# junhong-3dv/s2m2

Measured on AMD Instinct MI355X. Metric: stereo pairs/sec, S-model 1216x1024 fp16 refine_iter=3 (ms/pair = 1000*n_gpus/value), higher is better.
Workload: dtype f16; 1 GPU; S-model 1216x1024 refine_iter=3 use_positivity=True, 1 pair(s) per GPU per step, random-init weights (seeded LeCun normal); pairs_per_gpu=1, parallelism=dp1 (pairs sharded, RCCL gather of outputs to rank 0)

## Files before the change

### __graft_entry__.py

```python
import os
import sys

ROOT = os.path.dirname(os.path.abspath(__file__))
if ROOT not in sys.path:
    sys.path.insert(0, ROOT)


def build() -> None:
    from s2m2_amd.build import build as build_lib
    lib = build_lib(verbose=True)
    assert os.path.exists(lib)
    _check_isa()
    import s2m2_amd
    from s2m2_amd import hip
    hip.load()
    import oracle.s2m2_oracle
    _build_ref()
    print("[build] ok:", lib)


def _build_ref() -> None:
    from oracle import make_ref, ref_loader
    if os.path.isdir(make_ref.SRC):
        make_ref.build(verbose=True)
    print("[build] oracle/_ref:", "ok" if ref_loader.available() else f"absent ({ref_loader.why_not()})")


def _check_isa() -> None:
    from s2m2_amd import build as B
    csrc = os.path.join(ROOT, "s2m2_amd", "csrc")
    if "-DS2M2_UNTRACKED_LOADS=0" in B.effective_defines():
        print("[build] check_isa: skipped (tracked loads: nothing to guard)")
        return
    stamp = os.path.join(B.OBJ, f"check_isa.{B.config_key()}.ok")
    newest = max(os.path.getmtime(os.path.join(csrc, f)) for f in os.listdir(csrc) if f in ("conv.hip", "conv_narrow.hip", "fusion.hip", "ln_corr.hip", "convblock.hip", "convgru.hip") or f.endswith(".h"))
    newest = max(newest, os.path.getmtime(os.path.join(ROOT, "tools", "check_isa.py")))
    if os.path.exists(stamp) and os.path.getmtime(stamp) > newest:
        print("[build] check_isa: up to date")
        return
    import subprocess
    r = subprocess.run([sys.executable, os.path.join(ROOT, "tools", "check_isa.py")], capture_output=True, text=True)
    sys.stdout.write(r.stdout)
    if r.returncode != 0:
        if os.environ.get("S2M2_ISA_FALLBACK") == "1":
            print("[build] check_isa failed (assertions above): S2M2_ISA_FALLBACK=1 -> rebuilding with tracked loads (-DS2M2_UNTRACKED_LOADS=0)")
            B.build(force=True, verbose=True, extra_defines=("-DS2M2_UNTRACKED_LOADS=0",))
            return
        raise RuntimeError("tools/check_isa.py failed -- the violated assertions:\n" + r.stdout + r.stderr[-2000:] +
                           "\n(S2M2_ISA_FALLBACK=1 rebuilds the library with tracked loads instead of failing)")
    open(stamp, "w").write("ok\n")


def smoke() -> None:
    import torch
    from oracle import s2m2_oracle as O
    from s2m2_amd.model import S2M2
    from s2m2_amd.weights import seeded_state_dict, synthetic_pair
    assert torch.cuda.is_available(), "smoke() needs cuda:0"
    torch.cuda.set_device(0)
    sd = seeded_state_dict(128, 1, 1, 0)
    m = S2M2(128, 1, 1, use_positivity=True, refine_iter=1)
    m.load_state_dict(sd, strict=True)
    m = m.cuda().eval()
    left, right = synthetic_pair(64, 96, 1, 8, 0)
    cap = {}
    d, o, c = m(left.cuda(), right.cuda(), capture=cap)
    torch.cuda.synchronize()
    ocap = {}
# ... 17 lines not shown
```

### include/s2m2_hip.h

```cpp
#ifndef S2M2_HIP_H
#define S2M2_HIP_H

#include <stddef.h>
#include <stdint.h>

#ifdef __cplusplus
extern "C" {
#endif

enum { S2M2_F32 = 0, S2M2_F16 = 1 };

#define S2M2_ABI_VERSION 800
int s2m2_version(void);
const char* s2m2_last_error(void);
int s2m2_debug_poison_lds(void* stream);
int s2m2_debug_clock_probe(void* out, void* stream);

const char* s2m2_ln_corr_kernel_name(int C, int feat_dtype, int cv_dtype);

typedef struct s2m2_corr_desc {
    const void* tokens;
    const float* ln_weight;
    const float* ln_bias;
    void* cv;
// ... 160 lines not shown
    long long out_stride;
    int N, H, W, C;
    const void* w_conv0;
    const void* w_conv2;
    const void* w_1x0;
    const void* w_1x2;
    const float* b_conv0;
    const float* b_conv2;
    const float* b_1x0;
    const float* b_1x2;
    int patch_rows;
    int dtype;
} s2m2_convblock_desc;
int s2m2_conv_block_supported(int C, int H, int W, int dtype);
int s2m2_conv_block(const s2m2_convblock_desc* desc, void* stream);

typedef struct s2m2_convgru_desc {
    const void* h;
    long long h_stride;
    const void* x;
    long long x_stride;
    void* out;
    long long out_stride;
    int N, H, W, C;
    int KH, KW;
    const void* w_zr;
    const void* w_q;
    const float* b_zr;
    const float* b_q;
    int dtype;
} s2m2_convgru_desc;
int s2m2_conv_gru_supported(int C, int H, int W, int dtype);
int s2m2_conv_gru(const s2m2_convgru_desc* desc, void* stream);

typedef struct s2m2_pw_desc {
    const void* src[4];
    int src_c[4];
    long long src_stride[4];
    int nsrc;
    long long rows;
    const void* weight_frag;
    const float* bias;
    void* out;
    long long out_stride;
    int Cout;
    int act;
    int shuffle2, Ho, Wo;
    int dtype;
} s2m2_pw_desc;
int s2m2_pw_direct_supported(int K, int Cout, int dtype);
int s2m2_pw_direct(const s2m2_pw_desc* desc, void* stream);

typedef struct s2m2_narrow_desc {
    const void* x;
    long long x_stride;
    int N, H, W, Cin;
    const void* x1;
    long long x1_stride;
    int Cin1;
    const void* weight_frag;
    const float* bias;
    void* out;
    long long out_stride;
    int Cout, KH, KW, stride;
    int act;
    int dtype;
// ... 135 lines not shown
```

### s2m2_amd/csrc/plan.h

```cpp
#pragma once
#include <stddef.h>
#include <type_traits>
#include <vector>
#include "common.h"

namespace s2m2 {

bool plan_recording();
constexpr int kPlanMaskWords = 4;
struct PlanPtrMask {
    unsigned long long bits[kPlanMaskWords] = {0, 0, 0, 0};
    bool overflow = false;
    void set(size_t byte_off) {
        const size_t w = byte_off / 8;
        if (byte_off % 8 != 0 || w >= 64 * kPlanMaskWords) overflow = true;
        else bits[w / 64] |= 1ULL << (w % 64);
    }
    bool test(size_t w) const { return w < 64 * kPlanMaskWords && ((bits[w / 64] >> (w % 64)) & 1ULL) != 0; }
};
int plan_append(int (*tramp)(const void* blob, void* stream), const void* blob, size_t bytes, const char* name, const PlanPtrMask& mask);

struct PlanEntry {
    const char* name;
    int (*tramp)(const void* blob, void* stream);
// ... 60 lines not shown
}

template <typename D> struct PlanPtrFields;
#define S2M2_PLAN_PTRS(D, ...)                                                                                      \
    template <> struct PlanPtrFields<D> {                                                                           \
        static void mark(size_t base, PlanPtrMask& m) {                                                             \
            const size_t offs[] = {__VA_ARGS__};                                                                    \
            for (size_t o : offs) m.set(base + o);                                                                  \
        }                                                                                                           \
    };
#define S2M2_OFF(D, f) offsetof(D, f)
#define S2M2_OFF_I(D, f, i) (offsetof(D, f) + 8 * (i))
S2M2_PLAN_PTRS(s2m2_corr_desc, S2M2_OFF(s2m2_corr_desc, tokens), S2M2_OFF(s2m2_corr_desc, ln_weight), S2M2_OFF(s2m2_corr_desc, ln_bias),
               S2M2_OFF(s2m2_corr_desc, cv), S2M2_OFF(s2m2_corr_desc, start_event), S2M2_OFF(s2m2_corr_desc, stop_event))
S2M2_PLAN_PTRS(s2m2_conv_desc, S2M2_OFF_I(s2m2_conv_desc, src, 0), S2M2_OFF_I(s2m2_conv_desc, src, 1), S2M2_OFF_I(s2m2_conv_desc, src, 2),
               S2M2_OFF_I(s2m2_conv_desc, src, 3), S2M2_OFF(s2m2_conv_desc, weight), S2M2_OFF(s2m2_conv_desc, bias), S2M2_OFF(s2m2_conv_desc, out),
               S2M2_OFF(s2m2_conv_desc, aux0), S2M2_OFF(s2m2_conv_desc, aux1), S2M2_OFF(s2m2_conv_desc, ln_wsum), S2M2_OFF(s2m2_conv_desc, bias2))
S2M2_PLAN_PTRS(s2m2_chain_desc, S2M2_OFF(s2m2_chain_desc, x), S2M2_OFF(s2m2_chain_desc, res), S2M2_OFF(s2m2_chain_desc, out),
               S2M2_OFF_I(s2m2_chain_desc, weight, 0), S2M2_OFF_I(s2m2_chain_desc, weight, 1), S2M2_OFF_I(s2m2_chain_desc, weight, 2),
               S2M2_OFF_I(s2m2_chain_desc, bias, 0), S2M2_OFF_I(s2m2_chain_desc, bias, 1), S2M2_OFF_I(s2m2_chain_desc, bias, 2),
               S2M2_OFF_I(s2m2_chain_desc, ln_wsum, 0), S2M2_OFF_I(s2m2_chain_desc, ln_wsum, 1), S2M2_OFF_I(s2m2_chain_desc, ln_wsum, 2),
               S2M2_OFF(s2m2_chain_desc, ln_out), S2M2_OFF(s2m2_chain_desc, ln_gamma), S2M2_OFF(s2m2_chain_desc, ln_beta),
               S2M2_OFF(s2m2_chain_desc, fan_weight), S2M2_OFF(s2m2_chain_desc, fan_bias), S2M2_OFF(s2m2_chain_desc, fan_ln_wsum),
               S2M2_OFF(s2m2_chain_desc, fan_out))
S2M2_PLAN_PTRS(s2m2_rowattn_desc, S2M2_OFF(s2m2_rowattn_desc, x), S2M2_OFF(s2m2_rowattn_desc, out), S2M2_OFF(s2m2_rowattn_desc, weights),
               S2M2_OFF(s2m2_rowattn_desc, vectors), S2M2_OFF(s2m2_rowattn_desc, ln_out))
S2M2_PLAN_PTRS(s2m2_convblock_desc, S2M2_OFF(s2m2_convblock_desc, x), S2M2_OFF(s2m2_convblock_desc, out), S2M2_OFF(s2m2_convblock_desc, w_conv0),
               S2M2_OFF(s2m2_convblock_desc, w_conv2), S2M2_OFF(s2m2_convblock_desc, w_1x0), S2M2_OFF(s2m2_convblock_desc, w_1x2),
               S2M2_OFF(s2m2_convblock_desc, b_conv0), S2M2_OFF(s2m2_convblock_desc, b_conv2), S2M2_OFF(s2m2_convblock_desc, b_1x0),
               S2M2_OFF(s2m2_convblock_desc, b_1x2))
S2M2_PLAN_PTRS(s2m2_convgru_desc, S2M2_OFF(s2m2_convgru_desc, h), S2M2_OFF(s2m2_convgru_desc, x), S2M2_OFF(s2m2_convgru_desc, out),
               S2M2_OFF(s2m2_convgru_desc, w_zr), S2M2_OFF(s2m2_convgru_desc, w_q), S2M2_OFF(s2m2_convgru_desc, b_zr),
               S2M2_OFF(s2m2_convgru_desc, b_q))
S2M2_PLAN_PTRS(s2m2_pw_desc, S2M2_OFF_I(s2m2_pw_desc, src, 0), S2M2_OFF_I(s2m2_pw_desc, src, 1), S2M2_OFF_I(s2m2_pw_desc, src, 2),
               S2M2_OFF_I(s2m2_pw_desc, src, 3), S2M2_OFF(s2m2_pw_desc, weight_frag), S2M2_OFF(s2m2_pw_desc, bias), S2M2_OFF(s2m2_pw_desc, out))
S2M2_PLAN_PTRS(s2m2_narrow_desc, S2M2_OFF(s2m2_narrow_desc, x), S2M2_OFF(s2m2_narrow_desc, x1), S2M2_OFF(s2m2_narrow_desc, weight_frag),
               S2M2_OFF(s2m2_narrow_desc, bias), S2M2_OFF(s2m2_narrow_desc, out), S2M2_OFF(s2m2_narrow_desc, head_frag),
               S2M2_OFF(s2m2_narrow_desc, head_bias))

template <typename D> struct PlanDescBlob { int (*impl)(const D*, void*); D desc; };
template <typename D> int plan_desc_tramp(const void* blob, void* stream) {
    const auto* b = static_cast<const PlanDescBlob<D>*>(blob);
    return b->impl(&b->desc, stream);
}
template <typename D> int plan_dispatch_desc(const char* name, int (*impl)(const D*, void*), const D* d, void* stream) {
#if S2M2_RANGE_CHECK
    range_bind_tu();
    const int rc = impl(d, stream) || range_collect(name, stream);
#else
    const int rc = impl(d, stream);
#endif
    if (rc == 0 && d && plan_recording()) {
        PlanDescBlob<D> b;
        __builtin_memset(&b, 0, sizeof(b));
        b.impl = impl;
        b.desc = *d;
        PlanPtrMask m;
        PlanPtrFields<D>::mark(offsetof(PlanDescBlob<D>, desc), m);
        return plan_append(&plan_desc_tramp<D>, &b, sizeof(b), name, m);
    }
    return rc;
}

template <typename... T> struct TypeList {};
template <typename Done, typename... Rest> struct DropLast;
template <typename... D, typename L> struct DropLast<TypeList<D...>, L> { using type = TypeList<D...>; };
// ... 21 lines not shown
```

### s2m2_amd/engine.py

```python
from __future__ import annotations

import os
from dataclasses import dataclass
from functools import cached_property
from typing import Dict, Optional, Sequence, Tuple

import torch
import torch.nn.functional as F

from . import hip, pack

Tensor = torch.Tensor


@dataclass(eq=False)
class Layer:
    weight: Tensor
    bias: Optional[Tensor]
    kh: int
    kw: int
    cout: int
    korder: int = 0

    def __post_init__(self):
# ... 72 lines not shown
    return max(1, (MAX_PIXELS - 1) // (2 * H * W))


class Engine:
    def __init__(self, model, dtype: torch.dtype):
        hip.load()
        self.dtype = dtype
        self.C = model.feature_channels
        self.ntr = model.num_transformer
        self.use_positivity = model.use_positivity
        self.refine_iter = model.refine_iter
        self.output_upsample = model.output_upsample
        self.device = next(model.parameters()).device
        self.p: Dict[str, Tensor] = {n: q.detach().to(self.device, torch.float32) for n, q in model.named_parameters()}
        self._layers: Dict[object, Layer] = {}
        self._composites: Dict[object, object] = {}
        self._supported: Dict[tuple, object] = {}
        self._pe_cache: Dict[Tuple[int, int], Tuple[Tensor, Tensor]] = {}
        self._bufs: Dict[object, Tensor] = {}
        self._plans: Dict[object, object] = {}
        self._ns = None
        self.fuse_k1ln = os.environ.get("S2M2_FUSE_K1LN", "1") != "0"
        self.cv_band = 11 if (os.environ.get("S2M2_CV_BAND", "0") == "1" and self.use_positivity) else -1
        self.use_k12 = os.environ.get("S2M2_K12", "1") != "0"
        self.use_k12_head = self.use_k12 and os.environ.get("S2M2_K12_HEAD", "1") != "0"
        self.native_refine = os.environ.get("S2M2_REFINE_NATIVE", "1") != "0"
        self.use_rowfuse = os.environ.get("S2M2_ROWFUSE", "1") != "0"
        self.coarse_fuse = os.environ.get("S2M2_COARSE_FUSE", "1") != "0"
        self.use_convblock = os.environ.get("S2M2_CONVBLOCK", "1") != "0"
        self.convblock_maxpix = int(os.environ.get("S2M2_CONVBLOCK_MAXPIX", "40000"))
        self.convblock_c256 = os.environ.get("S2M2_CONVBLOCK_C256", "0") == "1"
        self.gru_frag = os.environ.get("S2M2_GRU_FRAG", "0") == "1"
        self.gru_fuse = os.environ.get("S2M2_GRU_FUSE", "1") != "0"
        self._tokens_normed: Optional[Tensor] = None
        self.ln_w = self.p["disp_init.layer_norm.weight"].contiguous()
        self.ln_b = self.p["disp_init.layer_norm.bias"].contiguous()
        self.k1_events = None

    def std(self, name: str, splits: Optional[Sequence[Tuple[int, int]]] = None, transposed: bool = False, frag: bool = True) -> Layer:
        key = (name, tuple(splits) if splits else None, transposed, bool(frag))
        s = self._layers.get(key)
        if s is None:
            w = self.p[name + ".weight"]
            if transposed:
                w = pack.convT_s1_as_conv(w)
            if w.dim() == 2:
                w = w[:, :, None, None]
            cin_p = sum(pd for _, pd in splits) if splits else pack.pad8(w.shape[1])
            frag = frag and pack.frag_eligible(pack.pad8(w.shape[0]), cin_p, w.shape[2], w.shape[3], self.dtype)
            wp = pack.pack_conv_frag(w, self.dtype, splits) if frag else pack.pack_conv(w, self.dtype, splits)
            s = self._layers[key] = Layer(wp, pack.pack_bias(self.p.get(name + ".bias"), w.shape[0]), w.shape[2], w.shape[3],
                                          pack.pad8(w.shape[0]), 2 if frag else 0)
        return s

    def merged(self, key: str, parts: Sequence[Tuple[str, int, float, bool]], cin_total: int) -> Layer:
        s = self._layers.get(key)
        if s is None:
            rows, biases = [], []
            kh = kw = 1
            for name, off, wscale, tr in parts:
                w = self.p[name + ".weight"]
                if tr:
                    w = pack.convT_s1_as_conv(w)
                if w.dim() == 2:
                    w = w[:, :, None, None]
                co, ci, kh, kw = w.shape
# ... 65 lines not shown
        b = self._bufs.get(k)
        if b is None:
            if self._ns is None and len(self._bufs) >= 64:
                self._bufs.pop(next(iter(self._bufs)))
            b = torch.zeros(shape, device=self.device, dtype=dtype or self.dtype)
            self._bufs[k] = b
        return b

    def down(self, p: str, x: Tensor) -> Tensor:
        spec = self.std(p + ".1")
        c = x.shape[-1]
        pooled = spec.is_1x1 and x.dim() == 4 and x.shape[1] >= 2 and x.shape[2] >= 2
        if pooled and (spec.plain_1x1(c, c) or spec.plain_1x1(c, 2 * c)) and self.chain_frag_ok(c):
            return hip.mlp_fan(x, *spec.fan(ln=False), pool2=True)
        if pooled:
            return self.cconv(spec, [x], pool2=True)
        return self.cconv(spec, [hip.resample2x(x, 0)])

    def up(self, p: str, x: Tensor) -> Tensor:
        spec = self.std(p + ".1")
        if spec.is_1x1:
            return hip.resample2x(self.cconv(spec, [x]), 1)
        return self.cconv(spec, [hip.resample2x(x, 1)])

    def conv_block(self, p: str, z: Tensor) -> Tensor:
        c0, c2 = self.std(p + ".convs_1x.0"), self.std(p + ".convs_1x.2")
        c = z.shape[-1]
        same = c0.cout == c and c2.cout == c
        if (self.use_convblock and same and z.dim() == 4 and z.shape[0] * z.shape[1] * z.shape[2] <= self.convblock_maxpix
                and (c == 128 or self.convblock_c256) and self.chain_frag_ok(c) and self.convblock_ok(c, z.shape[1], z.shape[2])):
            k0, k2 = self.std(p + ".convs.0"), self.std(p + ".convs.2")
            if k0.frag_3x3(c) and k2.frag_3x3(c) and c0.plain_1x1(c, c) and c2.plain_1x1(c, c):
                return hip.conv_block(z, k0.weight, k0.bias, k2.weight, k2.bias, c0.chain_frag, c0.bias, c2.chain_frag, c2.bias)
        if same and self.chain_frag_ok(c):
            b = hip.mlp_chain(z, [c0.stage(hip.ACT_RELU), c2.stage(hip.ACT_NONE)], frag=True)
        elif same and self.chain_ok(c):
            b = hip.mlp_chain(z, [c0.stage(hip.ACT_RELU, frag=False), c2.stage(hip.ACT_NONE, frag=False)])
        else:
            b = self.cconv(c2, [self.cconv(c0, [z], act=hip.ACT_RELU)])
        t = self.cconv(self.std(p + ".convs.0"), [z], act=hip.ACT_GELU)
        return self.cconv(self.std(p + ".convs.2"), [t], epi=hip.EPI_ADD, aux0=b)

    def gate_fusion(self, p: str, c: int) -> Layer:
        return self.merged(p + "|gate+fusion", [(p + ".feature_gate.0", 0, 1.0, False), (p + ".feature_fusion.0", 0, 1.0, False)], 2 * c)

    def dual_heads(self, p: str):
        def build():
            g2, f2 = self.std(p + ".feature_gate.2"), self.std(p + ".feature_fusion.2")
            return torch.cat([g2.weight, f2.weight], dim=1).contiguous(), g2.bias, f2.bias
        return self.composite(p + "|gate.2+fusion.2", build)

    def k10(self, p: str, z0: Tensor, z1: Tensor, first: Layer, z1_coarse: bool = False) -> Tensor:
        dual = self.dual_heads(p)
        if self.fusion_frag_ok(z0.shape[-1]):
            ws = self.composite(p + "|k10 fragment stream", lambda: pack.fusion_frag(first.weight, dual[0]))
            return hip.feature_fusion(z0, z1, ws, first.bias, None, dual[1], dual[2], z1_coarse=z1_coarse, frag=True)
        return hip.feature_fusion(z0, z1, first.weight, first.bias, dual[0], dual[1], dual[2], z1_coarse=z1_coarse)

    def fusion_up_ok(self, p: str, c: int, pu: str) -> bool:
        spec = self.std(pu + ".1")
        return (spec.is_1x1 and spec.cout == c and self.gate_fusion(p, c).is_1x1
                and self.p[p + ".feature_gate.0.weight"].shape[0] == c and self.fusion_ok(c))

    def up_tail(self, p: str, c_fine: int, pu: str, c_coarse: int) -> Optional[Layer]:
        spec = self.std(pu + ".1")
        if (self.coarse_fuse and self.fusion_up_ok(p, c_fine, pu) and spec.plain_1x1(c_coarse, c_coarse) and c_fine == c_coarse
# ... 12 lines not shown
        c = z0.shape[-1]
        cg = self.p[p + ".feature_gate.0.weight"].shape[0]
        spec = self.gate_fusion(p, c)
        if spec.is_1x1 and cg == c and self.fusion_ok(c):
            return self.k10(p, z0, z1, spec)
        gf = self.cconv(spec, [z0, z1], act=hip.ACT_GELU)
        if cg % 64 == 0:
            dual = self.dual_heads(p)
            return hip.conv2d([gf], dual[0], dual[1], 1, 1, dual[0].shape[0], act=hip.ACT_SIGMOID, epi=hip.EPI_DUALMIX, aux0=z0, aux1=z1,
                              ksplit=cg, bias2=dual[2])
        m = self.cconv(self.std(p + ".feature_gate.2"), [gf[..., :cg]], act=hip.ACT_SIGMOID, epi=hip.EPI_GATEMIX, aux0=z0, aux1=z1)
        return self.cconv(self.std(p + ".feature_fusion.2"), [gf[..., cg:]], epi=hip.EPI_ADD, aux0=m)

    def chain_ok(self, c: int) -> bool:
        return self.supported("mlp_chain", c)

    def chain_frag_ok(self, c: int) -> bool:
        return self.supported("mlp_chain_frag", c)

    def fusion_frag_ok(self, c: int) -> bool:
        return self.supported("feature_fusion_frag", c)

    def fusion_ok(self, c: int) -> bool:
        return self.supported("feature_fusion", c) or self.fusion_frag_ok(c)

    def pw_ok(self, k: int, cout: int) -> bool:
        return self.supported("pw_direct", k, cout)

    def narrow_ok(self, kh: int, kw: int, stride: int, cin: int, cout: int) -> bool:
        return self.use_k12 and self.supported("conv_narrow", kh, kw, stride, cin, cout)

    def gru_fuse_ok(self, c: int, h: int, w: int) -> bool:
        return getattr(hip, "conv_gru_supported", None) is not None and self.supported("conv_gru", c, h, w)

    def convblock_ok(self, c: int, h: int, w: int) -> bool:
        return self.supported("conv_block", c, h, w)

    def row_ok(self, z: Tensor, nh: int) -> bool:
        return self.use_rowfuse and z.dim() == 4 and self.supported("row_attn", z.shape[-1], nh, z.shape[2])

    def pe(self, h: int, w: int) -> Tuple[Tensor, Tensor]:
        key = (h, w)
        if key not in self._pe_cache:
            self._pe_cache[key] = pe_tables(h, w, self.device)
        return self._pe_cache[key]

    def qkv_spec(self, p: str) -> Layer:
        c = self.p[p + ".q.weight"].shape[1]
        return self.merged(p + "|qkv", [(p + ".q", 0, 1.0, False), (p + ".k", 0, 1.0, False), (p + ".v", 0, 1.0, False)], c)

    def qkv(self, p: str, x: Tensor) -> Tensor:
        spec = self.qkv_spec(p)
        c = x.shape[-1]
        if spec.is_1x1 and spec.cout == 3 * c and self.chain_frag_ok(c):
            return hip.mlp_fan(x, *spec.fan())
        return self.cconv(spec, [x], ln=True)

    def attn_core(self, p: str, z: Tensor, nh: int, two_d: bool, cross: bool, use_pe: bool, qkv: Optional[Tensor] = None) -> Tensor:
        n, h, w, c = z.shape
        if qkv is None:
            qkv = self.qkv(p + ".attn", z)
        v3 = qkv.reshape(n, h * w, 3 * c) if two_d else qkv.reshape(n * h, w, 3 * c)
        q, k, v = v3[..., :c], v3[..., c:2 * c], v3[..., 2 * c:]
        if use_pe:
            px, py = self.pe(h, w)
            o, pes = hip.attention(q, k, v, nh, pe=(px, py, w, h))
# ... 439 lines not shown
```

### s2m2_amd/hip.py

```python
from __future__ import annotations

import contextlib
import ctypes
import os
from typing import Optional, Tuple

import torch

_HERE = os.path.dirname(os.path.abspath(__file__))
LIB_PATH = os.path.join(_HERE, "lib", "libs2m2_hip%s.so" % os.environ.get("S2M2_LIB_SUFFIX", ""))

F32, F16 = 0, 1
_DT = {torch.float32: F32, torch.float16: F16}

_lib: Optional[ctypes.CDLL] = None

_vp, _i, _ll = ctypes.c_void_p, ctypes.c_int, ctypes.c_longlong

ACT_NONE, ACT_GELU, ACT_RELU, ACT_SIGMOID, ACT_TANH = 0, 1, 2, 3, 4
EPI_NONE, EPI_ADD, EPI_MUL, EPI_GRU, EPI_GATEMIX, EPI_DUALMIX = 0, 1, 2, 3, 4, 5


class ConvDesc(ctypes.Structure):
    _fields_ = [("src", _vp * 4), ("src_c", _i * 4), ("src_stride", _i * 4), ("nsrc", _i), ("weight", _vp), ("bias", _vp),
                ("out", _vp), ("out_stride", _i), ("N", _i), ("H", _i), ("W", _i), ("KH", _i), ("KW", _i), ("Cout", _i),
                ("act", _i), ("epi", _i), ("aux0", _vp), ("aux1", _vp), ("aux0_stride", _i), ("aux1_stride", _i),
                ("out_scale", ctypes.c_float), ("shuffle2", _i), ("tile", _i), ("dtype", _i), ("korder", _i), ("stride", _i),
                ("ln_wsum", _vp), ("ln_eps", ctypes.c_float), ("ksplit", _i), ("bias2", _vp), ("pool2", _i), ("epi_cout0", _i)]


class ChainDesc(ctypes.Structure):
    _fields_ = [("x", _vp), ("res", _vp), ("out", _vp), ("x_stride", _ll), ("res_stride", _ll), ("out_stride", _ll), ("rows", _ll),
                ("C", _i), ("nstage", _i), ("weight", _vp * 3), ("bias", _vp * 3), ("ln_wsum", _vp * 3), ("act", _i * 3),
                ("res_stage", _i), ("carry", _i), ("ln_eps", ctypes.c_float), ("dtype", _i),
                ("ln_out", _vp), ("ln_out_stride", _ll), ("ln_gamma", _vp), ("ln_beta", _vp), ("ln_out_eps", ctypes.c_float),
                ("fan_weight", _vp), ("fan_bias", _vp), ("fan_ln_wsum", _vp), ("fan_out", _vp), ("fan_out_stride", _ll),
                ("nfan", _i), ("xcd_group_rows", _ll), ("weight_frag", _i), ("pool_h", _i), ("pool_w", _i)]


class RowAttnDesc(ctypes.Structure):
    _fields_ = [("x", _vp), ("x_stride", _ll), ("out", _vp), ("out_stride", _ll), ("nimg", _i), ("h", _i), ("w", _i), ("C", _i), ("heads", _i),
                ("cross", _i), ("weights", _vp), ("vectors", _vp), ("ln_eps", ctypes.c_float),
                ("ln_out", _vp), ("ln_out_stride", _ll), ("ln_out_eps", ctypes.c_float), ("xcd_hint", _i), ("dtype", _i)]


class ConvBlockDesc(ctypes.Structure):
    _fields_ = [("x", _vp), ("x_stride", _ll), ("out", _vp), ("out_stride", _ll), ("N", _i), ("H", _i), ("W", _i), ("C", _i),
                ("w_conv0", _vp), ("w_conv2", _vp), ("w_1x0", _vp), ("w_1x2", _vp), ("b_conv0", _vp), ("b_conv2", _vp), ("b_1x0", _vp),
                ("b_1x2", _vp), ("patch_rows", _i), ("dtype", _i)]


class ConvGruDesc(ctypes.Structure):
    _fields_ = [("h", _vp), ("h_stride", _ll), ("x", _vp), ("x_stride", _ll), ("out", _vp), ("out_stride", _ll), ("N", _i), ("H", _i), ("W", _i),
                ("C", _i), ("KH", _i), ("KW", _i), ("w_zr", _vp), ("w_q", _vp), ("b_zr", _vp), ("b_q", _vp), ("dtype", _i)]


class PwDesc(ctypes.Structure):
    _fields_ = [("src", _vp * 4), ("src_c", _i * 4), ("src_stride", _ll * 4), ("nsrc", _i), ("rows", _ll), ("weight_frag", _vp), ("bias", _vp),
                ("out", _vp), ("out_stride", _ll), ("Cout", _i), ("act", _i), ("shuffle2", _i), ("Ho", _i), ("Wo", _i), ("dtype", _i)]


class NarrowDesc(ctypes.Structure):
    _fields_ = [("x", _vp), ("x_stride", _ll), ("N", _i), ("H", _i), ("W", _i), ("Cin", _i), ("x1", _vp), ("x1_stride", _ll), ("Cin1", _i),
                ("weight_frag", _vp), ("bias", _vp), ("out", _vp), ("out_stride", _ll), ("Cout", _i), ("KH", _i), ("KW", _i), ("stride", _i),
                ("act", _i), ("dtype", _i), ("head_frag", _vp), ("head_bias", _vp), ("head_cout", _i)]


class CorrDesc(ctypes.Structure):
    _fields_ = [("tokens", _vp), ("ln_weight", _vp), ("ln_bias", _vp), ("cv", _vp), ("B", _i), ("h", _i), ("w", _i), ("C", _i),
                ("cv_pitch", _i), ("band", _i), ("token_dtype", _i), ("cv_dtype", _i), ("start_event", _vp), ("stop_event", _vp)]


class PackDesc(ctypes.Structure):
    _fields_ = [("kind", _i), ("w", _vp), ("w2", _vp), ("rows", _i), ("cols", _i), ("ld", _i), ("ld2", _i), ("ntap", _i), ("out", _vp),
                ("out_elems", _ll)]


PACK_ROWS, PACK_NARROW, PACK_CONV_FRAG, PACK_FUSION, PACK_HEAD = range(5)

REGION_CONTENT, REGION_SCRATCH, REGION_EXTERNAL = range(3)


class EngineRegion(ctypes.Structure):
    _fields_ = [("base", _vp), ("bytes", ctypes.c_ulonglong), ("kind", _i)]


class EngineInfo(ctypes.Structure):
# ... 44 lines not shown
    "s2m2_plan_end": (_i, [_vp, ctypes.POINTER(_vp), ctypes.POINTER(ctypes.c_size_t), _i]),
    "s2m2_plan_abort": (_i, [_vp]),
    "s2m2_plan_launches": (_i, [_vp]),
    "s2m2_plan_patches": (_i, [_vp, _i]),
    "s2m2_plan_run": (_i, [_vp, ctypes.POINTER(_vp), _i, _vp]),
    "s2m2_plan_destroy": (_i, [_vp]),
    "s2m2_refine_step": (_i, [_vp, _vp, _vp, _vp, _vp, _vp, _vp, _vp, _vp]),
    "s2m2_plan_save": (_i, [_vp, ctypes.POINTER(EngineRegion), _i, ctypes.POINTER(EngineInfo), ctypes.c_char_p]),
    "s2m2_engine_load": (_i, [ctypes.c_char_p, ctypes.POINTER(_vp)]),
    "s2m2_engine_meta": (_i, [_vp, ctypes.POINTER(EngineInfo)]),
    "s2m2_engine_run": (_i, [_vp, _vp, _vp, _vp, _vp, _vp, _vp]),
    "s2m2_engine_destroy": (_i, [_vp]),
    "s2m2_pack_frag_elems": (_ll, [ctypes.POINTER(PackDesc)]),
    "s2m2_pack_frag": (_i, [ctypes.POINTER(PackDesc), _vp]),
    "s2m2_event_create": (_i, [ctypes.POINTER(_vp)]),
    "s2m2_event_destroy": (_i, [_vp]),
    "s2m2_event_elapsed_us": (_i, [_vp, _vp, ctypes.POINTER(ctypes.c_float)]),
    "s2m2_sinkhorn_workspace_bytes": (ctypes.c_size_t, [_i, _i, _i, _i]),
    "s2m2_pw_direct_supported": (_i, [_i, _i, _i]),
    "s2m2_pw_direct": (_i, [ctypes.POINTER(PwDesc), _vp]),
    "s2m2_conv_narrow_supported": (_i, [_i, _i, _i, _i, _i, _i]),
    "s2m2_conv_narrow": (_i, [ctypes.POINTER(NarrowDesc), _vp]),
    "s2m2_sinkhorn_regress": (_i, [_vp, _vp, _vp, _vp, _vp, _i, _i, _i, _i, _i, _i, _i, _vp, _vp]),
    "s2m2_cv_lookup": (_i, [_vp, _vp, _vp, _vp, _i, _i, _i, _i, _i, _i, _ll, _ll, _ll, _i, _vp]),
    "s2m2_conv2d": (_i, [ctypes.POINTER(ConvDesc), _vp]),
    "s2m2_mlp_chain_supported": (_i, [_i, _i]),
    "s2m2_mlp_chain_frag_supported": (_i, [_i, _i]),
    "s2m2_mlp_fan_supported": (_i, [_i, _i, _i]),
    "s2m2_mlp_chain": (_i, [ctypes.POINTER(ChainDesc), _vp]),
    "s2m2_conv_block_supported": (_i, [_i, _i, _i, _i]),
    "s2m2_conv_block": (_i, [ctypes.POINTER(ConvBlockDesc), _vp]),
    "s2m2_conv_gru_supported": (_i, [_i, _i, _i, _i]),
    "s2m2_conv_gru": (_i, [ctypes.POINTER(ConvGruDesc), _vp]),
    "s2m2_row_attn_supported": (_i, [_i, _i, _i, _i]),
    "s2m2_row_attn": (_i, [ctypes.POINTER(RowAttnDesc), _vp]),
    "s2m2_feature_fusion_supported": (_i, [_i, _i]),
    "s2m2_feature_fusion": (_i, [_vp, _vp, _vp, _ll, _ll, _ll, _ll, _i, _vp, _vp, _vp, _vp, _vp, _i, _i, _i, _vp]),
    "s2m2_feature_fusion_frag_supported": (_i, [_i, _i]),
    "s2m2_feature_fusion_frag": (_i, [_vp, _vp, _vp, _ll, _ll, _ll, _ll, _i, _vp, _vp, _vp, _vp, _i, _i, _i, _vp]),
    "s2m2_convex_upsample": (_i, [_vp, _vp, _vp, _i, _vp, _i, _i, _i, _i, _i, _i, _vp, _ll, _i, _vp]),
    "s2m2_attention": (_i, [_vp, _vp, _vp, _vp, _ll, _ll, _ll, _ll, _i, _i, _i, _i, _i, ctypes.c_float, _i, _vp, _vp, _vp, _ll,
                            _i, _i, _i, _vp]),
    "s2m2_attention_supported": (_i, [_i, _i, _i, _i, _i, _i, _i]),
    "s2m2_resample2x": (_i, [_vp, _vp, _i, _i, _i, _i, _ll, _ll, _i, _i, _vp]),
    "s2m2_image_prep": (_i, [_vp, _vp, _vp, _i, _i, _i, _i, _i, _vp]),
    "s2m2_refine_prep": (_i, [_vp, _vp, _vp, _vp, _ll, _i, _i, _vp]),
    "s2m2_global_update": (_i, [_vp, _i, _vp, _vp, _vp, _ll, _i, _i, _vp]),
    "s2m2_refine_update": (_i, [_vp, _i, _vp, _vp, _vp, _ll, _i, _i, _i, _vp]),
    "s2m2_debug_poison_lds": (_i, [_vp]),
    "s2m2_debug_clock_probe": (_i, [_vp, _vp]),
    "s2m2_refine_update_to": (_i, [_vp, _i, _vp, _vp, _vp, _vp, _vp, _vp, _vp, _ll, _i, _i, _i, _vp]),
    "s2m2_tanh": (_i, [_vp, _vp, _ll, _i, _vp]),
    "s2m2_stem_mlp": (_i, [_vp, _vp, _vp, _vp, _vp, _vp, _ll, _i, _vp]),
    "s2m2_image_pad": (_i, [_vp, _vp, _vp, _i, _i, _i, _i, _i, _i, _vp]),
    "s2m2_layernorm": (_i, [_vp, _vp, _ll, _i, _ll, _ll, _i, _vp]),
    "s2m2_groupnorm_workspace_bytes": (ctypes.c_size_t, [_i, _i]),
    "s2m2_groupnorm_nhwc": (_i, [_vp, _vp, _vp, _vp, _vp, _i, _ll, _i, _i, ctypes.c_float, _i, _vp]),
    "s2m2_cloud_workspace_bytes": (ctypes.c_size_t, [_i, _i, _i]),
    "s2m2_cloud": (_i, [ctypes.POINTER(CloudDesc), _vp]),
    "s2m2_rectify": (_i, [ctypes.POINTER(RectifyDesc), _vp]),
    "s2m2_eval_workspace_bytes": (ctypes.c_size_t, [_i, _i, _i]),
    "s2m2_eval_tile_rows": (_i, [_i, _i]),
    "s2m2_disp_eval": (_i, [ctypes.POINTER(EvalDesc), _vp]),
}


# ... 879 lines not shown
    if s0.dim() == 3 and s0.dtype == torch.uint8 and s0.shape[2] == 3:
        fmt, (Hs, Ws) = RECTIFY_SRC_U8_HWC, s0.shape[:2]
    elif s0.dim() == 3 and s0.shape[0] == 3 and s0.dtype in (torch.uint8, torch.float32):
        fmt, (Hs, Ws) = RECTIFY_SRC_U8_CHW if s0.dtype == torch.uint8 else RECTIFY_SRC_F32_CHW, s0.shape[1:]
    else:
        raise ValueError("rectify: a source is an (H,W,3) uint8, (3,H,W) uint8 or (3,H,W) fp32 tensor")
    if records.dtype != torch.float32 or records.dim() != 2 or records.shape[1] != RECTIFY_RECORD_FLOATS or records.shape[0] < 1:
        raise ValueError(f"rectify: records must be an (n_img, {RECTIFY_RECORD_FLOATS}) fp32 tensor")
    n = records.shape[0]
    if out is None and maps is None:
        raise ValueError("rectify: no output requested")
    ref = out if out is not None else maps
    if ref.dim() != 4:
        raise ValueError("rectify: out is (n_img,3,Hd,Wd), maps is (n_img,2,Hd,Wd)")
    Hd, Wd = (hd, wd) if hd is not None and wd is not None else ref.shape[-2:]
    d = RectifyDesc()
    if out is not None:
        if out.dtype not in (torch.float32, torch.uint8):
            raise ValueError("rectify: out must be an (n_img,3,Hd,Wd) fp32 or uint8 tensor")
        _mat(out, (n, 3, Hd, Wd), out.dtype, "rectify: out")
        d.out, d.out_dtype = out.data_ptr(), _IMG_DT[out.dtype]
        d.src[0], d.src[1] = srcs[0].data_ptr(), srcs[-1].data_ptr()
    if maps is not None:
        _mat(maps, (n, 2, Hd, Wd), torch.float32, "rectify: maps")
        d.maps = maps.data_ptr()
    d.records, d.n_src, d.n_img, d.Hs, d.Ws, d.Hd, d.Wd = records.data_ptr(), len(srcs), n, Hs, Ws, Hd, Wd
    d.src_format, d.round, d.order = fmt, int(bool(round)), order
    with torch.cuda.device(records.device):
        _check(load().s2m2_rectify(ctypes.byref(d), _stream()), "s2m2_rectify")


from .hip_gru import conv_gru, conv_gru_supported
from .hip_eval import disp_eval, eval_tile_rows, eval_workspace_bytes
```

Before: 129.2 pairs/s.

## Fuse conv block tail: second 3x3 conv, 1x1 MLP branch and residual add

Adds a HIP kernel that takes the GELU output of the first 3x3 conv plus the block input. In one launch per tile it runs the 1x1 ReLU/1x1 MLP branch on the input, the second 3x3 conv over a halo tile, and the sum of the two, keeping intermediates in LDS and registers. This replaces separate conv and mlp_chain launches and their intermediate global-memory round trips. It is enabled by default for C=128 and picks the patch shape with an occupancy heuristic. The cost is a large LDS footprint and a new code path that must match the prior numerics.

```diff
diff --git a/__graft_entry__.py b/__graft_entry__.py
--- a/__graft_entry__.py
+++ b/__graft_entry__.py
@@ -33,7 +33,7 @@
         print("[build] check_isa: skipped (tracked loads: nothing to guard)")
         return
     stamp = os.path.join(B.OBJ, f"check_isa.{B.config_key()}.ok")
-    newest = max(os.path.getmtime(os.path.join(csrc, f)) for f in os.listdir(csrc) if f in ("conv.hip", "conv_narrow.hip", "fusion.hip", "ln_corr.hip", "convblock.hip", "convgru.hip") or f.endswith(".h"))
+    newest = max(os.path.getmtime(os.path.join(csrc, f)) for f in os.listdir(csrc) if f in ("conv.hip", "conv_narrow.hip", "fusion.hip", "ln_corr.hip", "convblock.hip", "convgru.hip", "convtail.hip") or f.endswith(".h"))
     newest = max(newest, os.path.getmtime(os.path.join(ROOT, "tools", "check_isa.py")))
     if os.path.exists(stamp) and os.path.getmtime(stamp) > newest:
         print("[build] check_isa: up to date")
diff --git a/include/s2m2_hip.h b/include/s2m2_hip.h
--- a/include/s2m2_hip.h
+++ b/include/s2m2_hip.h
@@ -216,6 +216,26 @@
 } s2m2_convgru_desc;
 int s2m2_conv_gru_supported(int C, int H, int W, int dtype);
 int s2m2_conv_gru(const s2m2_convgru_desc* desc, void* stream);
+
+typedef struct s2m2_convtail_desc {
+    const void* t;
+    long long t_stride;
+    const void* z;
+    long long z_stride;
+    void* out;
+    long long out_stride;
+    int N, H, W, C;
+    const void* w_conv2;
+    const void* w_1x0;
+    const void* w_1x2;
+    const float* b_conv2;
+    const float* b_1x0;
+    const float* b_1x2;
+    int patch_rows, patch_cols;
+    int dtype;
+} s2m2_convtail_desc;
+int s2m2_conv_block_tail_supported(int C, int H, int W, int dtype);
+int s2m2_conv_block_tail(const s2m2_convtail_desc* desc, void* stream);
 
 typedef struct s2m2_pw_desc {
     const void* src[4];
diff --git a/s2m2_amd/csrc/convtail.hip b/s2m2_amd/csrc/convtail.hip
--- /dev/null
+++ b/s2m2_amd/csrc/convtail.hip
@@ -0,0 +1,293 @@
+#include "common.h"
+#include "launch.h"
+#include "plan.h"
+#include "epilogue.h"
+#include "frag_ring.h"
+#include "convtail_select.h"
+#include <stdint.h>
+
+namespace s2m2 {
+
+struct CtArgs {
+    const half_t* t; const half_t* z; half_t* out;
+    unsigned ts, zs, os;
+    int N, H, W, tiles_x, tiles_y;
+    const raw16_t* w2;
+    const raw16_t* wa; const raw16_t* wb;
+    const float* b2; const float* ba; const float* bb;
+    const void* zero;
+};
+
+template <int C_, int PH_, int PW_>
+struct CtCfg {
+    static constexpr int C = C_, PH = PH_, PW = PW_, NW = C_ / 32, NT = 64 * NW, KS = 8, CH = 128, NCHUNK = C_ / 128;
+    static constexpr int NP = PH * PW, MT = NP / 32;
+    static constexpr int HH = PH + 2, HW = PW + 2, NHALO = HH * HW;
+    static constexpr int RS = CH + 8, TRS = C + 8;
+    static constexpr int PPX = CH / 8, RPI = NT / PPX, A_IT = (NHALO + RPI - 1) / RPI, AROWS = A_IT * RPI;
+    static constexpr size_t A_BYTES = (size_t)AROWS * RS * 2;
+    static constexpr size_t Z_BYTES = (size_t)NP * TRS * 2;
+    static constexpr size_t OFF_B = ((A_BYTES > Z_BYTES ? A_BYTES : Z_BYTES) + 15) / 16 * 16, LDS_BYTES = OFF_B + 3 * C * 4;
+    static constexpr int ZP = C / 8, SP = NP * ZP / NT;
+    static_assert(NP % 32 == 0 && NP * ZP % NT == 0 && NT % PPX == 0 && LDS_BYTES <= 160 * 1024, "conv block tail tile");
+    static_assert(C != 128 || LDS_BYTES <= 80 * 1024, "C = 128: two blocks per CU");
+};
+
+template <typename CFG>
+__device__ __forceinline__ void tail_1x1(float16_t (&acc)[CFG::MT], const half_t* tile, const raw16_t* wf, int l31, int hi) {
+    constexpr int KS = CFG::KS, MT = CFG::MT;
+#pragma unroll
+    for (int i = 0; i < MT; ++i)
+#pragma unroll
+        for (int r = 0; r < 16; ++r) acc[i][r] = 0.f;
+#pragma unroll 1
+    for (int c8 = 0; c8 < CFG::C / 16; c8 += KS) {
+        raw16_t wr[KS];
+#pragma unroll
+        for (int s = 0; s < KS; ++s) wr[s] = global_load16(wf + (size_t)(c8 + s) * 64);
+#pragma unroll
+        for (int s = 0; s < KS; ++s) {
+            Frag<half_t> wfr;
+            wfr.v = __builtin_bit_cast(half8_t, wr[s]);
+#pragma unroll
+            for (int i = 0; i < MT; ++i) {
+                Frag<half_t> xf;
+                load_frag(xf, tile + (size_t)(32 * i + l31) * CFG::TRS + hi * 8 + (c8 + s) * 16);
+                mma32(acc[i], wfr, xf);
+            }
+        }
+    }
+}
+
+template <typename CFG>
+__global__ __launch_bounds__(CFG::NT, 2) void conv_tail_kernel(CtArgs p) {
+    constexpr int C = CFG::C, PW = CFG::PW, KS = CFG::KS, RS = CFG::RS, TRS = CFG::TRS, HW = CFG::HW, MT = CFG::MT, NCHUNK = CFG::NCHUNK;
+    extern __shared__ __attribute__((aligned(16))) char smem[];
+    half_t* Zt = reinterpret_cast<half_t*>(smem);
+    half_t* Ah = reinterpret_cast<half_t*>(smem);
+    float* bvec = reinterpret_cast<float*>(smem + CFG::OFF_B);
+    const int tid = threadIdx.x, lane = tid & 63, l31 = lane & 31, hi = lane >> 5;
+    const int wv = __builtin_amdgcn_readfirstlane(tid >> 6);
+    int bx = blockIdx.x;
+    const int tx = bx % p.tiles_x; bx /= p.tiles_x;
+    const int ty = bx % p.tiles_y;
+    const int n = bx / p.tiles_y;
+    const int y0 = ty * CFG::PH, x0 = tx * PW;
+    const half_t* zp = static_cast<const half_t*>(p.zero);
+
+    for (int i = tid; i < 3 * C; i += CFG::NT) {
+        const int k = i / C, c = i - k * C;
+        const float* src = k == 0 ? p.b2 : k == 1 ? p.ba : p.bb;
+        bvec[i] = src ? src[c] : 0.f;
+    }
+    auto piece_pix = [&](int t, int it) __attribute__((always_inline)) -> int {
+        const int r = (t + CFG::NT * it) / CFG::ZP;
+        const int py = r / PW, yy = y0 + py, xx = x0 + (r - py * PW);
+        return (yy < p.H && xx < p.W) ? (n * p.H + yy) * p.W + xx : -1;
+    };
+    {
+        raw16_t rz[CFG::SP];
+#pragma unroll
+        for (int it = 0; it < CFG::SP; ++it) {
+            const int s = tid + CFG::NT * it, r = s / CFG::ZP, pcc = s - r * CFG::ZP;
+            const int m = piece_pix(tid, it);
+            rz[it] = global_load16(m >= 0 ? p.z + ((unsigned)m * p.zs + pcc * 8) : zp);
+        }
+#pragma unroll
+        for (int it = 0; it < CFG::SP; ++it) {
+            const int s = tid + CFG::NT * it, r = s / CFG::ZP, pcc = s - r * CFG::ZP;
+            *reinterpret_cast<raw16_t*>(Zt + (size_t)r * TRS + pcc * 8) = rz[it];
+        }
+    }
+    __syncthreads();
+
+    unsigned s1[MT][8];
+    {
+        float16_t accA[MT];
+        tail_1x1<CFG>(accA, Zt, p.wa + (size_t)wv * (C / 16) * 64 + lane, l31, hi);
+        __syncthreads();
+#pragma unroll
+        for (int i = 0; i < MT; ++i) {
+            half_t* rrow = Zt + (size_t)(32 * i + l31) * TRS + wv * 32 + 4 * hi;
+#pragma unroll
+            for (int gq = 0; gq < 4; ++gq) {
+                const float4_t bv = *reinterpret_cast<const float4_t*>(bvec + C + wv * 32 + 8 * gq + 4 * hi);
+                half4_t h;
+#pragma unroll
+                for (int e = 0; e < 4; ++e) h[e] = from_f32<half_t>(fmaxf(accA[i][4 * gq + e] + bv[e], 0.f) * 1.0f);
+                *reinterpret_cast<half4_t*>(rrow + 8 * gq) = h;
+            }
+        }
+        __syncthreads();
+        float16_t accB[MT];
+        tail_1x1<CFG>(accB, Zt, p.wb + (size_t)wv * (C / 16) * 64 + lane, l31, hi);
+#pragma unroll
+        for (int i = 0; i < MT; ++i)
+#pragma unroll
+            for (int gq = 0; gq < 4; ++gq) {
+                const float4_t bv = *reinterpret_cast<const float4_t*>(bvec + 2 * C + wv * 32 + 8 * gq + 4 * hi);
+#pragma unroll
+                for (int e = 0; e < 4; e += 2) {
+                    const half2_t pr = {from_f32<half_t>((accB[i][4 * gq + e] + bv[e]) * 1.0f), from_f32<half_t>((accB[i][4 * gq + e + 1] + bv[e + 1]) * 1.0f)};
+                    unsigned u = __builtin_bit_cast(unsigned, pr);
+                    asm volatile("" : "+v"(u));
+                    s1[i][2 * gq + e / 2] = u;
+                }
+            }
+    }
+    __syncthreads();
+
+    auto load_halo = [&](int chunk) __attribute__((always_inline)) {
+        int t = tid;
+        asm volatile("" : "+v"(t));
+        const int pc = t % CFG::PPX, prow = t / CFG::PPX;
+        raw16_t ra[CFG::A_IT];
+#pragma unroll
+        for (int it = 0; it < CFG::A_IT; ++it) {
+            const int hp = prow + CFG::RPI * it;
+            const int hy = hp / HW, hx = hp - hy * HW;
+            const int yy = y0 - 1 + hy, xx = x0 - 1 + hx;
+            const bool ok = hp < CFG::NHALO && yy >= 0 && yy < p.H && xx >= 0 && xx < p.W;
+            const half_t* src = ok ? p.t + ((unsigned)((n * p.H + yy) * p.W + xx) * p.ts + chunk * CFG::CH + pc * 8) : zp;
+            ra[it] = global_load16(src);
+        }
+#pragma unroll
+        for (int it = 0; it < CFG::A_IT; ++it) *reinterpret_cast<raw16_t*>(Ah + (size_t)(prow + CFG::RPI * it) * RS + pc * 8) = ra[it];
+    };
+    const int nfrag = NCHUNK * 9 * KS;
+    const raw16_t* wf = p.w2 + (size_t)wv * nfrag * 64 + lane;
+    raw16_t ring[KS];
+#pragma unroll
+    for (int s = 0; s < KS - 1; ++s) global_load16_async(ring[s], wf + (size_t)s * 64);
+    load_halo(0);
+    __syncthreads();
+    float16_t acc[MT];
+#pragma unroll
+    for (int i = 0; i < MT; ++i)
+#pragma unroll
+        for (int r = 0; r < 16; ++r) acc[i][r] = 0.f;
+    int poff[MT];
+#pragma unroll
+    for (int i = 0; i < MT; ++i) {
+        const int q = 32 * i + l31, qy = q / PW;
+        poff[i] = (qy * HW + (q - qy * PW)) * RS + hi * 8;
+    }
+    int g = 0;
+#pragma unroll 1
+    for (int chunk = 0; chunk < NCHUNK; ++chunk) {
+        if (chunk > 0) {
+            wait_vmcnt<0>();
+            __syncthreads();
+            load_halo(chunk);
+            __syncthreads();
+        }
+        int ky = 0, kx = 0;
+#pragma unroll 1
+        for (int tap = 0; tap < 9; ++tap) {
+            cb_steps<MT, KS>(acc, Ah + (ky * HW + kx) * RS, poff, ring, wf, g, nfrag);
+            if (++kx == 3) { kx = 0; ++ky; }
+        }
+    }
+    wait_vmcnt<0>();
+#pragma unroll
+    for (int s = 0; s < KS; ++s) settle(ring[s]);
+    __syncthreads();
+
+#pragma unroll
+    for (int i = 0; i < MT; ++i) {
+        half_t* srow = Zt + (size_t)(32 * i + l31) * TRS + wv * 32 + 4 * hi;
+#pragma unroll
+        for (int gq = 0; gq < 4; ++gq) {
+            const float4_t b2 = *reinterpret_cast<const float4_t*>(bvec + wv * 32 + 8 * gq + 4 * hi);
+            half4_t h;
+#pragma unroll
+            for (int e = 0; e < 4; ++e) {
+                const half_t m = from_f32<half_t>((acc[i][4 * gq + e] + b2[e]) * 1.0f);
+                h[e] = from_f32<half_t>((float)m + (float)__builtin_bit_cast(half2_t, s1[i][2 * gq + e / 2])[e & 1]);
+            }
+            *reinterpret_cast<half4_t*>(srow + 8 * gq) = h;
+        }
+    }
+    __syncthreads();
+    int tid_s = tid;
+    asm volatile("" : "+v"(tid_s));
+#pragma unroll
+    for (int it = 0; it < CFG::SP; ++it) {
+        const int s = tid_s + CFG::NT * it, r = s / CFG::ZP, pcc = s - r * CFG::ZP;
+        const int m = piece_pix(tid_s, it);
+        if (m < 0) continue;
+        *reinterpret_cast<raw16_t*>(p.out + ((unsigned)m * p.os + pcc * 8)) = *reinterpret_cast<const raw16_t*>(Zt + (size_t)r * TRS + pcc * 8);
+    }
+}
+
+template <int C, int PH, int PW>
+static int launch_ct(const CtArgs& a0, hipStream_t st) {
+    using CFG = CtCfg<C, PH, PW>;
+    CtArgs a = a0;
+    a.tiles_x = (a.W + PW - 1) / PW;
+    a.tiles_y = (a.H + PH - 1) / PH;
+    return launch<conv_tail_kernel<CFG>>("conv_block_tail", dim3((unsigned)(a.N * a.tiles_x * a.tiles_y)), dim3(CFG::NT), CFG::LDS_BYTES, st, a);
+}
+
+template <int C>
+static int launch_ct_patch(const CtArgs& a, hipStream_t st, ConvTailPatch pt) {
+    if (pt.pw == 40) return launch_ct<C, 4, 40>(a, st);
+    return pt.ph == 4 ? launch_ct<C, 4, 32>(a, st) : launch_ct<C, 2, 32>(a, st);
+}
+
+static int tail_tensor(const char* name, const void* ptr, long long stride, long long pixels, int C) {
+    S2M2_REQUIRE(ptr, "conv_block_tail: %s is null", name);
+    S2M2_REQUIRE((uintptr_t)ptr % 16 == 0, "conv_block_tail: %s must be 16-byte aligned", name);
+    S2M2_REQUIRE(stride >= C && stride % 8 == 0, "conv_block_tail: %s_stride=%lld (at least C = %d and a multiple of 8)", name, stride, C);
+    S2M2_REQUIRE(pixels * stride < (1LL << 31), "conv_block_tail: %s spans 2^31 elements or more", name);
+    return 0;
+}
+static int tail_weight(const char* name, const void* ptr) {
+    S2M2_REQUIRE(ptr, "conv_block_tail: %s is null", name);
+    S2M2_REQUIRE((uintptr_t)ptr % 16 == 0, "conv_block_tail: %s must be 16-byte aligned", name);
+    return 0;
+}
+static int tail_disjoint(const char* name, const void* in, long long in_stride, const void* out, long long out_stride, long long pixels, int C) {
+    const uintptr_t a0 = (uintptr_t)in, a1 = a0 + (size_t)((pixels - 1) * in_stride + C) * 2;
+    const uintptr_t o0 = (uintptr_t)out, o1 = o0 + (size_t)((pixels - 1) * out_stride + C) * 2;
+    S2M2_REQUIRE(o1 <= a0 || a1 <= o0, "conv_block_tail: out aliases %s", name);
+    return 0;
+}
+
+}
+
+extern "C" int s2m2_conv_block_tail_supported(int C, int H, int W, int dtype) {
+    return dtype == S2M2_F16 && (C == 128 || C == 256) && H >= 1 && W >= 1;
+}
+
+static int conv_block_tail_impl(const s2m2_convtail_desc* d, void* stream) {
+    using namespace s2m2;
+    S2M2_REQUIRE(d, "conv_block_tail: null descriptor");
+    S2M2_REQUIRE(d->dtype == S2M2_F16, "conv_block_tail: dtype=%d (fp16 only)", d->dtype);
+    S2M2_REQUIRE(d->C == 128 || d->C == 256, "conv_block_tail: C=%d (128 or 256)", d->C);
+    S2M2_REQUIRE(d->N > 0 && d->H > 0 && d->W > 0 && (long long)d->N * d->H * d->W < (1LL << 24), "conv_block_tail: bad shape");
+    const long long pixels = (long long)d->N * d->H * d->W;
+    if (tail_tensor("t", d->t, d->t_stride, pixels, d->C) || tail_tensor("z", d->z, d->z_stride, pixels, d->C) ||
+        tail_tensor("out", d->out, d->out_stride, pixels, d->C)) return 1;
+    if (tail_weight("w_conv2", d->w_conv2) || tail_weight("w_1x0", d->w_1x0) || tail_weight("w_1x2", d->w_1x2)) return 1;
+    if (tail_disjoint("t", d->t, d->t_stride, d->out, d->out_stride, pixels, d->C) ||
+        tail_disjoint("z", d->z, d->z_stride, d->out, d->out_stride, pixels, d->C)) return 1;
+    const bool forced = d->patch_rows != 0 || d->patch_cols != 0;
+    const ConvTailPatch pt = conv_tail_patch(d->N, d->H, d->W, d->C, d->patch_rows, d->patch_cols);
+    S2M2_REQUIRE(!forced || (pt.ph == d->patch_rows && pt.pw == d->patch_cols), "conv_block_tail: patch %d x %d (2 x 32, 4 x 32 or 4 x 40)",
+                 d->patch_rows, d->patch_cols);
+    CtArgs a;
+    a.t = static_cast<const half_t*>(d->t); a.z = static_cast<const half_t*>(d->z); a.out = static_cast<half_t*>(d->out);
+    a.ts = (unsigned)d->t_stride; a.zs = (unsigned)d->z_stride; a.os = (unsigned)d->out_stride;
+    a.N = d->N; a.H = d->H; a.W = d->W;
+    a.w2 = static_cast<const raw16_t*>(d->w_conv2); a.wa = static_cast<const raw16_t*>(d->w_1x0); a.wb = static_cast<const raw16_t*>(d->w_1x2);
+    a.b2 = d->b_conv2; a.ba = d->b_1x0; a.bb = d->b_1x2;
+    if (bind_zero_page(a, "conv_block_tail")) return 1;
+    hipStream_t st = static_cast<hipStream_t>(stream);
+    return d->C == 256 ? launch_ct_patch<256>(a, st, pt) : launch_ct_patch<128>(a, st, pt);
+}
+static constexpr char kConvTailEntry[] = "s2m2_conv_block_tail";
+extern "C" int s2m2_conv_block_tail(const s2m2_convtail_desc* d, void* stream) {
+    return s2m2::plan_dispatch_desc<s2m2_convtail_desc>(kConvTailEntry, &conv_block_tail_impl, d, stream);
+}
+S2M2_PLAN_DESC_ENTRY(kConvTailEntry, conv_block_tail_impl)
diff --git a/s2m2_amd/csrc/convtail_select.h b/s2m2_amd/csrc/convtail_select.h
--- /dev/null
+++ b/s2m2_amd/csrc/convtail_select.h
@@ -0,0 +1,19 @@
+#pragma once
+
+namespace s2m2 {
+
+struct ConvTailPatch {
+    int ph, pw;
+};
+
+inline ConvTailPatch conv_tail_patch(int N, int H, int W, int C, int force_ph = 0, int force_pw = 0) {
+    if ((force_ph == 2 && force_pw == 32) || (force_ph == 4 && (force_pw == 32 || force_pw == 40))) return {force_ph, force_pw};
+    const long long slots = 512, small = 256, per_patch = C / 128;
+    const long long b4 = (long long)N * ((W + 31) / 32) * ((H + 3) / 4) * per_patch;
+    const long long b5 = (long long)N * ((W + 39) / 40) * ((H + 3) / 4) * per_patch;
+    const long long cost4 = ((b4 + slots - 1) / slots) * 4, cost5 = ((b5 + slots - 1) / slots) * 5;
+    if (b4 > small && cost5 < cost4 + 4) return {4, 40};
+    return {2, 32};
+}
+
+}
diff --git a/s2m2_amd/csrc/plan.h b/s2m2_amd/csrc/plan.h
--- a/s2m2_amd/csrc/plan.h
+++ b/s2m2_amd/csrc/plan.h
@@ -116,6 +116,9 @@
 S2M2_PLAN_PTRS(s2m2_convgru_desc, S2M2_OFF(s2m2_convgru_desc, h), S2M2_OFF(s2m2_convgru_desc, x), S2M2_OFF(s2m2_convgru_desc, out),
                S2M2_OFF(s2m2_convgru_desc, w_zr), S2M2_OFF(s2m2_convgru_desc, w_q), S2M2_OFF(s2m2_convgru_desc, b_zr),
                S2M2_OFF(s2m2_convgru_desc, b_q))
+S2M2_PLAN_PTRS(s2m2_convtail_desc, S2M2_OFF(s2m2_convtail_desc, t), S2M2_OFF(s2m2_convtail_desc, z), S2M2_OFF(s2m2_convtail_desc, out),
+               S2M2_OFF(s2m2_convtail_desc, w_conv2), S2M2_OFF(s2m2_convtail_desc, w_1x0), S2M2_OFF(s2m2_convtail_desc, w_1x2),
+               S2M2_OFF(s2m2_convtail_desc, b_conv2), S2M2_OFF(s2m2_convtail_desc, b_1x0), S2M2_OFF(s2m2_convtail_desc, b_1x2))
 S2M2_PLAN_PTRS(s2m2_pw_desc, S2M2_OFF_I(s2m2_pw_desc, src, 0), S2M2_OFF_I(s2m2_pw_desc, src, 1), S2M2_OFF_I(s2m2_pw_desc, src, 2),
                S2M2_OFF_I(s2m2_pw_desc, src, 3), S2M2_OFF(s2m2_pw_desc, weight_frag), S2M2_OFF(s2m2_pw_desc, bias), S2M2_OFF(s2m2_pw_desc, out))
 S2M2_PLAN_PTRS(s2m2_narrow_desc, S2M2_OFF(s2m2_narrow_desc, x), S2M2_OFF(s2m2_narrow_desc, x1), S2M2_OFF(s2m2_narrow_desc, weight_frag),
diff --git a/s2m2_amd/engine.py b/s2m2_amd/engine.py
--- a/s2m2_amd/engine.py
+++ b/s2m2_amd/engine.py
@@ -128,6 +128,8 @@
         self.convblock_c256 = os.environ.get("S2M2_CONVBLOCK_C256", "0") == "1"
         self.gru_frag = os.environ.get("S2M2_GRU_FRAG", "0") == "1"
         self.gru_fuse = os.environ.get("S2M2_GRU_FUSE", "1") != "0"
+        self.cb_tail = os.environ.get("S2M2_CB_TAIL", "1") != "0"
+        self.cb_tail_c256 = os.environ.get("S2M2_CB_TAIL_C256", "0") == "1"
         self._tokens_normed: Optional[Tensor] = None
         self.ln_w = self.p["disp_init.layer_norm.weight"].contiguous()
         self.ln_b = self.p["disp_init.layer_norm.bias"].contiguous()
@@ -259,6 +261,12 @@
             k0, k2 = self.std(p + ".convs.0"), self.std(p + ".convs.2")
             if k0.frag_3x3(c) and k2.frag_3x3(c) and c0.plain_1x1(c, c) and c2.plain_1x1(c, c):
                 return hip.conv_block(z, k0.weight, k0.bias, k2.weight, k2.bias, c0.chain_frag, c0.bias, c2.chain_frag, c2.bias)
+        if (self.cb_tail and same and z.dim() == 4 and (c == 128 or self.cb_tail_c256) and self.chain_frag_ok(c)
+                and self.cb_tail_ok(c, z.shape[1], z.shape[2])):
+            k0, k2 = self.std(p + ".convs.0"), self.std(p + ".convs.2")
+            if k0.frag_3x3(c) and k2.frag_3x3(c) and c0.plain_1x1(c, c) and c2.plain_1x1(c, c):
+                t = self.cconv(k0, [z], act=hip.ACT_GELU)
+                return hip.conv_block_tail(t, z, k2.weight, k2.bias, c0.chain_frag, c0.bias, c2.chain_frag, c2.bias)
         if same and self.chain_frag_ok(c):
             b = hip.mlp_chain(z, [c0.stage(hip.ACT_RELU), c2.stage(hip.ACT_NONE)], frag=True)
         elif same and self.chain_ok(c):
@@ -337,6 +345,9 @@
 
     def gru_fuse_ok(self, c: int, h: int, w: int) -> bool:
         return getattr(hip, "conv_gru_supported", None) is not None and self.supported("conv_gru", c, h, w)
+
+    def cb_tail_ok(self, c: int, h: int, w: int) -> bool:
+        return getattr(hip, "conv_block_tail_supported", None) is not None and self.supported("conv_block_tail", c, h, w)
 
     def convblock_ok(self, c: int, h: int, w: int) -> bool:
         return self.supported("conv_block", c, h, w)
diff --git a/s2m2_amd/hip.py b/s2m2_amd/hip.py
--- a/s2m2_amd/hip.py
+++ b/s2m2_amd/hip.py
@@ -53,6 +53,12 @@
 class ConvGruDesc(ctypes.Structure):
     _fields_ = [("h", _vp), ("h_stride", _ll), ("x", _vp), ("x_stride", _ll), ("out", _vp), ("out_stride", _ll), ("N", _i), ("H", _i), ("W", _i),
                 ("C", _i), ("KH", _i), ("KW", _i), ("w_zr", _vp), ("w_q", _vp), ("b_zr", _vp), ("b_q", _vp), ("dtype", _i)]
+
+
+class ConvTailDesc(ctypes.Structure):
+    _fields_ = [("t", _vp), ("t_stride", _ll), ("z", _vp), ("z_stride", _ll), ("out", _vp), ("out_stride", _ll), ("N", _i), ("H", _i), ("W", _i),
+                ("C", _i), ("w_conv2", _vp), ("w_1x0", _vp), ("w_1x2", _vp), ("b_conv2", _vp), ("b_1x0", _vp), ("b_1x2", _vp), ("patch_rows", _i),
+                ("patch_cols", _i), ("dtype", _i)]
 
 
 class PwDesc(ctypes.Structure):
@@ -163,6 +169,8 @@
     "s2m2_conv_block": (_i, [ctypes.POINTER(ConvBlockDesc), _vp]),
     "s2m2_conv_gru_supported": (_i, [_i, _i, _i, _i]),
     "s2m2_conv_gru": (_i, [ctypes.POINTER(ConvGruDesc), _vp]),
+    "s2m2_conv_block_tail_supported": (_i, [_i, _i, _i, _i]),
+    "s2m2_conv_block_tail": (_i, [ctypes.POINTER(ConvTailDesc), _vp]),
     "s2m2_row_attn_supported": (_i, [_i, _i, _i, _i]),
     "s2m2_row_attn": (_i, [ctypes.POINTER(RowAttnDesc), _vp]),
     "s2m2_feature_fusion_supported": (_i, [_i, _i]),
@@ -1108,3 +1116,5 @@
 
 from .hip_gru import conv_gru, conv_gru_supported
 from .hip_eval import disp_eval, eval_tile_rows, eval_workspace_bytes
+
+from .hip_tail import conv_block_tail, conv_block_tail_supported
diff --git a/s2m2_amd/hip_tail.py b/s2m2_amd/hip_tail.py
--- /dev/null
+++ b/s2m2_amd/hip_tail.py
@@ -0,0 +1,39 @@
+import ctypes
+from typing import Optional, Tuple
+
+import torch
+
+from . import hip as _h
+
+
+def conv_block_tail_supported(C: int, H: int, W: int, dtype: torch.dtype) -> bool:
+    return bool(_h.load().s2m2_conv_block_tail_supported(C, H, W, _h._DT[dtype]))
+
+
+def conv_block_tail(t: torch.Tensor, z: torch.Tensor, w_conv2: torch.Tensor, b_conv2, w_1x0: torch.Tensor, b_1x0, w_1x2: torch.Tensor, b_1x2,
+                    out: Optional[torch.Tensor] = None, patch: Optional[Tuple[int, int]] = None) -> torch.Tensor:
+    _h._resident("conv_block_tail", t, z, w_conv2, b_conv2, w_1x0, b_1x0, w_1x2, b_1x2, out)
+    if t.dtype != torch.float16 or z.dtype != torch.float16 or tuple(t.shape) != tuple(z.shape):
+        raise ValueError("conv_block_tail: t and z must be (N,H,W,C) fp16 tensors of one shape")
+    ts, zs = _h._pixels(t, "conv_block_tail: t"), _h._pixels(z, "conv_block_tail: z")
+    N, H, W, C = t.shape
+    if out is None:
+        out = torch.empty((N, H, W, C), device=t.device, dtype=t.dtype)
+    elif out.dtype != t.dtype or tuple(out.shape) != tuple(t.shape):
+        raise ValueError("conv_block_tail: out must be an fp16 tensor of t's shape")
+    os_ = _h._pixels(out, "conv_block_tail: out")
+    _h._vec(w_conv2, 9 * C * C, "conv_block_tail: w_conv2", dtype=t.dtype)
+    _h._vec(w_1x0, C * C, "conv_block_tail: w_1x0", dtype=t.dtype)
+    _h._vec(w_1x2, C * C, "conv_block_tail: w_1x2", dtype=t.dtype)
+    for name, b in (("b_conv2", b_conv2), ("b_1x0", b_1x0), ("b_1x2", b_1x2)):
+        _h._vec(b, C, f"conv_block_tail: {name}", optional=True)
+    d = _h.ConvTailDesc()
+    d.t, d.t_stride, d.z, d.z_stride, d.out, d.out_stride = t.data_ptr(), ts, z.data_ptr(), zs, out.data_ptr(), os_
+    d.N, d.H, d.W, d.C = N, H, W, C
+    d.w_conv2, d.w_1x0, d.w_1x2 = w_conv2.data_ptr(), w_1x0.data_ptr(), w_1x2.data_ptr()
+    d.b_conv2, d.b_1x0, d.b_1x2 = _h._ptr(b_conv2), _h._ptr(b_1x0), _h._ptr(b_1x2)
+    d.patch_rows, d.patch_cols = patch if patch is not None else (0, 0)
+    d.dtype = _h._DT[t.dtype]
+    _h._check(_h.load().s2m2_conv_block_tail(ctypes.byref(d), _h._stream()), "s2m2_conv_block_tail")
+    _h._meter("conv_block_tail", 2.0 * N * H * W * C * C * 11)
+    return out
```

Measured after the change: 132.6 pairs/s, median of 6. +2.6%, better.
